# emrullahArkun/tinycarlo

Measured on AMD Instinct MI355X. Metric: env-steps/sec (whole node), higher is better.
Workload: dtype f64; 1 GPU; cfg3: 4096 envs/GPU, simple_layout map, 64x64 'classes' obs, with camera laneline raster; envs_per_gpu=4096, steps_per_launch=128, entry_point=tc_step_multi, observations=every step's frame stored to its own row of a [128, N, ...] rollout buffer, preroll_steps=1024, calls_prepared=True, actions=v~U(0.3,1) s~U(-1,1) maneuver~U{0..3}/64 steps, on device, autoreset=True, spawn=host queue (reference seed parity), resets_since_queue_top_up=18375, max_respawns_of_one_env_since_top_up=11, spawn_queue_len=64, max_segments_per_frame=49, frames_sampled=196608, on_road_term=False, lds_bytes_per_env=9760

## Files before the change

### tinycarlo_amd/csrc/k_common.h

```cpp
#ifndef K_COMMON_H
#define K_COMMON_H

#include <hip/hip_runtime.h>

#include "../../include/tinycarlo_hip.h"
#include "k_probe.h"
#include "tc_cull.h"
#include "tc_device.h"

#if defined(TC_PART) && defined(TC_DEV_FAST)
#error "the development builds are one translation unit"
#endif
#if defined(TC_PART) && TC_PART > 0
#define TC_PLAIN_KERNEL static
#else
#define TC_PLAIN_KERNEL
#endif

#define TC_PROF_RING 64
#define TC_RING_SLOTS 3
#define MODE_STEP 0
#define MODE_RESET 1
#define MODE_RENDER 2

__device__ __forceinline__ void lds_sync() { asm volatile("s_waitcnt lgkmcnt(0)" ::: "memory"); }

template <class T>
__device__ __forceinline__ const T& kernarg_again(const T& r) {
  unsigned long long p = (unsigned long long)&r;
  asm volatile("" : "+s"(p));
  return *(const T*)(const __attribute__((address_space(4))) T*)p;
}

#define RB_MAX 32
#define RB_OF_K(K) ((K) >= 8 ? 16 : 32)
#define R_OFF_TAB 0
#define R_TAB_BYTES_OF(RB) (((RB) * 4 * 5 + (RB) * 4 + 5 * (RB) + 8 * (RB)) * 4 + 2 * 4 * (RB) * 8)
#define R_OFF_BITS_OF(RB) ((R_TAB_BYTES_OF(RB) + 15) / 16 * 16)
#define R_OFF_LC_OF(RB) ((RB) * 116)
#define R_TAB_BYTES_SH(RB, sh) (R_OFF_LC_OF(RB) + ((RB) << (sh)) * (4 + 5 * 4))
#define R_OFF_BITS_SH(RB, sh) ((R_TAB_BYTES_SH(RB, sh) + 15) / 16 * 16)
static_assert(R_TAB_BYTES_SH(32, 2) == R_TAB_BYTES_OF(32) && R_TAB_BYTES_SH(16, 2) == R_TAB_BYTES_OF(16), "the four-edge form is the full size");
#define LCH 8

#define TC_MAX_GROUPS 8
struct LdsLayout {
  int off_p, off_flg, off_list, off_cnt;
  int total;
  int off_live;
};

struct LiveLds {
  double d[10];
  double cte, he, reward;
  double dist[TC_MAX_LAYERS];
  int lp[8];
  int lp_len, last_maneuver;
  int have_trig;
  int needs_reset;
  int cursor;
  int cursor0;
  int trunc, status, terminated;
  int ep_len;
  int cam_idx;
  int pad;
  int cnt[TC_MAX_TERMS];
  int ne[TC_MAX_LAYERS];
  double ep_ret;
};
#define TC_LIVE_BYTES 416
static_assert(sizeof(LiveLds) <= TC_LIVE_BYTES, "LiveLds must fit its LDS slot");

struct RollStep {
  double *reward, *cte, *heading_error;
  unsigned char *terminated, *truncated;
  int* status;
  double *x, *y, *theta, *velocity;
  double* dist;
  int* ne;
  int* lp;
  int* lp_len;
  size_t row0;
};

struct KArgs {
  DevMap m;
  DevCar car;
  DevCam cam;
  tc_buffers b;
  LdsLayout lds;
  int N;
  int env0;
  const double* cam_E;
  const double* cam_K;
  int* seg_g;
  int* seg_n;
  int seg_cap;
  const tc_term* terms;
  int n_terms;
  int* term_counters;
  int n_grp;
  int grp_layer[TC_MAX_GROUPS + 1];
  int grp_n0[TC_MAX_GROUPS + 1], grp_e0[TC_MAX_GROUPS + 1];
  int grp_l0[TC_MAX_GROUPS], grp_l1[TC_MAX_GROUPS];
  const double2* cam_nodes;
  const int2* cam_edges_g;
  int cap_nodes;
  const int* spawn_tab;
  int spawn_n;
  unsigned long long spawn_seed;
  unsigned int dbg;
  int seg_lds_off, seg_lds_cap;
  int clip_merge;
  int frame_cull;
  int cull_rows;
  const unsigned char* cull_tab;
  TcCullCover cull;
};

__device__ __forceinline__ double d_readlane(double v, int l) {
  const int lo = __builtin_amdgcn_readlane(__double2loint(v), l);
  const int hi = __builtin_amdgcn_readlane(__double2hiint(v), l);
  return __hiloint2double(hi, lo);
}

__device__ __forceinline__ int uni_i(int v) { return __builtin_amdgcn_readfirstlane(v); }
__device__ __forceinline__ double uni_d(double v) {
  const int lo = __builtin_amdgcn_readfirstlane(__double2loint(v));
  const int hi = __builtin_amdgcn_readfirstlane(__double2hiint(v));
  return __hiloint2double(hi, lo);
}

typedef __attribute__((address_space(3))) int* LdsIntPtr;

__device__ __forceinline__ int wave_rank(unsigned long long m) {
  return (int)__builtin_amdgcn_mbcnt_hi((unsigned)(m >> 32), __builtin_amdgcn_mbcnt_lo((unsigned)m, 0u));
}

__device__ inline unsigned int spread4(unsigned int x) {
  const unsigned int m = (x * 0x00204081u) & 0x01010101u;
  return (m << 8) - m;
}

__device__ __forceinline__ int wave_incl_scan(int v, int lane) {
  (void)lane;
  v += __builtin_amdgcn_update_dpp(0, v, 0x111, 0xf, 0xf, true);
  v += __builtin_amdgcn_update_dpp(0, v, 0x112, 0xf, 0xf, true);
  v += __builtin_amdgcn_update_dpp(0, v, 0x114, 0xf, 0xf, true);
  v += __builtin_amdgcn_update_dpp(0, v, 0x118, 0xf, 0xf, true);
  v += __builtin_amdgcn_update_dpp(0, v, 0x142, 0xa, 0xf, false);
  v += __builtin_amdgcn_update_dpp(0, v, 0x143, 0xc, 0xf, false);
  return v;
}

struct MultiArgs {
  int nsteps;
  int seg_rows;
  int cam_here;
  double* pose_rows;
  unsigned int* resident;
  int map_lds;
  int fat_lds;
  int grp_off, grp_stride, cnt_off;
  tc_rollout roll;
};
__device__ __forceinline__ RollStep roll_at(const tc_rollout& r, size_t row0, int C) {
  RollStep q;
  q.reward = r.reward;
  q.cte = r.cte;
  q.heading_error = r.heading_error;
  q.terminated = r.terminated;
  q.truncated = r.truncated;
  q.status = r.status;
  q.x = r.x;
  q.y = r.y;
  q.theta = r.theta;
  q.velocity = r.velocity;
  q.dist = r.laneline_distances;
  q.ne = r.nearest_edge;
  q.lp = r.local_path;
  q.lp_len = r.lp_len;
  q.row0 = row0;
  return q;
}

#endif
```

### tinycarlo_amd/csrc/k_raster.h

```cpp
#ifndef K_RASTER_H
#define K_RASTER_H

#include "k_common.h"
#include "tc_device.h"
#include "tc_rng.h"

struct RCam {
  int H, W, wpr, band_rows, n_bands, thickness, format;
  int cap_r;
  unsigned char cap_hw[32];
  unsigned int cap_hw4;
};
struct RArgs {
  int N, C;
  int env0;
  RCam cam;
  unsigned char colors[16][3];
  const int* seg_g;
  const int* seg_n;
  int seg_cap;
  unsigned char* obs;
  const unsigned char* mask;
  int off_tab, off_bits;
  unsigned int flags;
  int seg_row0;
  int noise_row0;
  long long obs_row_stride;
  int noise_blobs, noise_max_radius;
  const unsigned char* noise_hw;
  unsigned long long noise_seed;
  const unsigned int* noise_step;
  int seg_lds_off, seg_lds_cap;
  unsigned int colors_packed[16];
};

#ifndef TC_RASTER_WAVES
#define TC_RASTER_WAVES 4
#endif
#ifndef TC_BAND_VMCNT
#define TC_BAND_VMCNT 0
#endif
#define TC_BAND_THROTTLE() asm volatile("s_waitcnt vmcnt(%0)" ::"n"(TC_BAND_VMCNT) : "memory")
__host__ __device__ __forceinline__ size_t tc_obs_bytes_of(int fmt, int C, int H, int W) {
  return fmt == TC_FMT_CLASSES_BITS ? (size_t)C * H * (size_t)(W >> 3) : (size_t)H * W * (fmt == TC_FMT_CLASSES ? C : 3);
}
#define TC_FMT_IS_CLASSES(fmt) ((fmt) == TC_FMT_CLASSES || (fmt) == TC_FMT_CLASSES_BITS)
__device__ __forceinline__ void packed_zero_words(unsigned char* dst, const int nw, const int tid) {
  if ((((unsigned long long)dst) & 15ull) == 0) {
    const int n4 = nw >> 2;
    const uint4 z = make_uint4(0, 0, 0, 0);
    for (int q = tid; q < n4; q += TC_NT) ((uint4*)dst)[q] = z;
    for (int i = (n4 << 2) + tid; i < nw; i += TC_NT) ((unsigned int*)dst)[i] = 0u;
  } else {
    for (int i = tid; i < nw; i += TC_NT) ((unsigned int*)dst)[i] = 0u;
  }
}
__device__ __forceinline__ void packed_copy_words(unsigned char* dst, const unsigned int* src, const int src_word0, const int nw,
                                                  const int tid) {
  if ((((unsigned long long)dst) & 15ull) == 0 && (src_word0 & 3) == 0) {
    const int n4 = nw >> 2;
    for (int q = tid; q < n4; q += TC_NT) ((uint4*)dst)[q] = ((const uint4*)src)[q];
    for (int i = (n4 << 2) + tid; i < nw; i += TC_NT) ((unsigned int*)dst)[i] = src[i];
  } else {
    for (int i = tid; i < nw; i += TC_NT) ((unsigned int*)dst)[i] = src[i];
  }
}
template <bool THICK, int FMT, bool LDSONLY = false, int RB = RB_MAX, bool FORM = false, bool ONE_BAND = false>
__device__ __forceinline__ void raster_body(const RArgs& a0, unsigned char* smem, int env, unsigned char* obs_base,
                                            const int tid, const size_t seg_slot0, const int nseg_in,
                                            const unsigned int used_in, const int frame_row) {
  const RArgs& a = a0;
  const RCam& cam = a.cam;
  auto n_bands_of = [](const RCam& c) { return ONE_BAND ? 1 : c.n_bands; };
  unsigned int* bits = (unsigned int*)(smem + (FORM ? a.off_bits : R_OFF_BITS_OF(RB)));
  const int* segg = a.seg_g + (seg_slot0 + env) * a.seg_cap * 5;
  const LdsIntPtr seg_lds = (LdsIntPtr)(smem + a.seg_lds_off);
  const int seg_lds_cap = a.seg_lds_cap;
  struct SegV {
    int v[5];
    __device__ __forceinline__ int operator[](int i) const { return v[i]; }
  };
  int lds_base = 0;
  const bool refill = LDSONLY && nseg_in > seg_lds_cap;
  const int rb_step = (refill && seg_lds_cap < RB) ? seg_lds_cap : RB;
  auto seg_refill = [&](int base, int nb) {
    lds_sync();
    for (int i = threadIdx.x; i < 5 * nb; i += TC_NT) seg_lds[i] = segg[5 * base + i];
    lds_base = base;
    lds_sync();
  };
  auto seg_get = [&](int k) {
    SegV r;
    if (LDSONLY) {
#pragma unroll
      for (int i = 0; i < 5; i++) r.v[i] = seg_lds[5 * (k - lds_base) + i];
    } else if (k < seg_lds_cap) {
#pragma unroll
      for (int i = 0; i < 5; i++) r.v[i] = seg_lds[5 * k + i];
    } else {
#pragma unroll
      for (int i = 0; i < 5; i++) r.v[i] = segg[5 * k + i];
    }
    return r;
  };
  auto seg_layer = [&](int k) { return LDSONLY ? seg_lds[5 * (k - lds_base)] : k < seg_lds_cap ? seg_lds[5 * k] : segg[5 * k]; };
  int nseg = nseg_in;
  unsigned int used_layers = used_in;
  TSTAMP(8);
  if (!LDSONLY && nseg_in < 0) {
    nseg = a.seg_n[seg_slot0 + env];
    used_layers = 0;
    for (int k = tid; k < nseg; k += TC_NT) used_layers |= 1u << segg[5 * k];
#pragma unroll
    for (int off = 32; off > 0; off >>= 1) used_layers |= __shfl_xor(used_layers, off);
  }

  int H = cam.H, W = cam.W, wpr = cam.wpr, C = a.C;
  constexpr bool CLS = TC_FMT_IS_CLASSES(FMT), BITS = FMT == TC_FMT_CLASSES_BITS;
  unsigned char* out = obs_base + (size_t)env * tc_obs_bytes_of(FMT, C, H, W);
  int* lt0 = (int*)(smem + R_OFF_TAB);
  int* lc0 = lt0 + RB * 4 * 5;
  int* fl = FORM ? (int*)(smem + R_OFF_TAB) : lc0 + RB * 4;
  int* fc = fl + RB;
  int* fm = fc + RB;
  int* fd = fm + RB;
  int* fpy = fd + 2 * RB;
  int* fpv = fpy + 4 * RB;
  long long* fpx = (long long*)(fpv + 4 * RB);
  long long* fpd = fpx + 4 * RB;
  static_assert(R_OFF_LC_OF(RB) == 13 * RB * 4 + 2 * 4 * RB * 8 && (13 * RB * 4) % 8 == 0, "FORM: lc starts where the fixed tables end");
  unsigned int early_zero = 0;
  if (CLS && n_bands_of(cam) == 1 && (W & 15) == 0 && a.noise_blobs == 0 && !DBG_ON(a.flags, DBG_SKIP_STORE)) {
    const int per_plane = H * (W >> 4);
    const uint4 zero4 = make_uint4(0, 0, 0, 0);
    for (int c = 0; c < C; c++) {
      if ((used_layers >> c) & 1u) continue;
      if (BITS) {
        packed_zero_words(out + (size_t)c * H * wpr * 4, H * wpr, tid);
        continue;
      }
      uint4* po = (uint4*)(out + (size_t)c * H * W);
      for (int q = tid; q < per_plane; q += TC_NT) po[q] = zero4;
    }
    early_zero = ~used_layers;
    if (nseg == 0) {
      TSTAMP(9);
      TSTAMP(10);
      TSTAMP(11);
      TSTAMP(12);
      TSTAMP(13);
      TSTAMP_REAL(31);
      return;
    }
  }
  for (int band = 0; band < n_bands_of(cam); band++) {
    if constexpr (FORM && !ONE_BAND) {
      const RArgs& ab = kernarg_again(a0);
      H = ab.cam.H, W = ab.cam.W, wpr = ab.cam.wpr, C = ab.C;
    }
    const int y0 = band * cam.band_rows;
    const int y1 = (y0 + cam.band_rows < H) ? y0 + cam.band_rows : H;
    const int rows = y1 - y0;
    const int nwords = C * cam.band_rows * wpr;
    if (n_bands_of(cam) > 1 && (W & 15) == 0) {
      bool touched = refill;
      const long long mg = (long long)cam.thickness + 2;
      for (int k0 = 0; k0 < nseg && !touched; k0 += TC_NT) {
        bool t = false;
        if (k0 + tid < nseg) {
          const SegV sg = seg_get(k0 + tid);
          const long long ya = sg[2], yb = sg[4];
          t = (ya < yb ? yb : ya) + mg >= y0 && (ya < yb ? ya : yb) - mg < y1;
        }
        touched = __ballot(t) != 0;
      }
      if (!touched && DBG_ON(a.flags, DBG_SKIP_STORE)) continue;
      if (!touched) {
        const uint4 z = make_uint4(0, 0, 0, 0);
        TC_BAND_THROTTLE();
        if (BITS) {
          for (int c = 0; c < C; c++) packed_zero_words(out + ((size_t)c * H + y0) * wpr * 4, rows * wpr, tid);
        } else if (CLS) {
          const int per_plane = rows * (W >> 4);
          for (int c = 0; c < C; c++) {
            uint4* dst = (uint4*)(out + ((size_t)c * H + y0) * W);
            for (int q = tid; q < per_plane; q += TC_NT) dst[q] = z;
          }
        } else {
          const int n16 = rows * W * 3 / 16;
          uint4* dst = (uint4*)(out + (size_t)y0 * W * 3);
          for (int q = tid; q < n16; q += TC_NT) dst[q] = z;
        }
        continue;
      }
    }
    {
      const int n4 = nwords >> 2;
      for (int i = tid; i < n4; i += TC_NT) ((uint4*)bits)[i] = make_uint4(0, 0, 0, 0);
      for (int i = (n4 << 2) + tid; i < nwords; i += TC_NT) bits[i] = 0;
    }
    lds_sync();
    TSTAMP(9);
#ifdef TC_TIMING_LDS
    TSTAMP(26);
#endif
    Ras r;
    r.W = W;
    r.H = H;
    r.wpr = wpr;
    r.y0 = y0;
    r.y1 = y1;
    const int plane = cam.band_rows * wpr;
    if (DBG_ON(a.flags, DBG_SKIP_RASTER)) {
    } else if (!THICK) {
      for (int base = 0; base < nseg; base += refill ? rb_step : nseg) {
        const int nb = refill ? (nseg - base < rb_step ? nseg - base : rb_step) : nseg;
        if (refill) seg_refill(base, nb);
        for (int k = base + tid; k < base + nb; k += TC_NT) {
          const SegV sg = seg_get(k);
          r.bits = bits + sg[0] * plane;
          r_line_bresenham(r, sg[1], sg[2], sg[3], sg[4]);
        }
      }
    } else {
      for (int base = 0; base < nseg; base += rb_step) {
        const RArgs& a = kernarg_again(a0);
        const RCam& cam = a.cam;
        const int nb = nseg - base < rb_step ? nseg - base : rb_step;
        if (refill) seg_refill(base, nb);
#ifdef TC_TIMING_LDS
        if (cam.n_bands >= 0) TSTAMP(27);
#endif
        if (n_bands_of(cam) > 1) {
          bool t = false;
          if (tid < nb) {
            const SegV sg = seg_get(base + tid);
            const long long ya = sg[2], yb = sg[4], mg = (long long)cam.thickness + 2;
            t = (ya < yb ? yb : ya) + mg >= y0 && (ya < yb ? ya : yb) - mg < y1;
          }
          if (__ballot(t) == 0) continue;
        }
#ifdef TC_TIMING_LDS
        if (cam.thickness > 0) TSTAMP(24);
#endif
        if (tid < RB) {
          int nrow = 0, lo = 0, np = 0, wm = 0, dpx = 0, dpy = 0, okq = 0;
#ifdef TC_TIMING_LDS
          TSTAMP(25);
#endif
          if (tid < nb) {
            const SegV sg = seg_get(base + tid);
            long long qx0, qx1, qx2, qx3, qy0, qy1, qy2, qy3;
            TSTAMP(20);
            bool touch = true;
            if (n_bands_of(cam) > 1) {
              const long long ya = sg[2], yb = sg[4], mg = (long long)cam.thickness + 2;
              const long long ymin = (ya < yb ? ya : yb) - mg, ymax = (ya < yb ? yb : ya) + mg;
              touch = ymax >= y0 && ymin < y1;
            }
            if (touch && !DBG_ON(a.flags, DBG_SKIP_QUAD) && r_quad_dp(sg[1], sg[2], sg[3], sg[4], cam.thickness, dpx, dpy)) {
              TSTAMP(21);
              okq = 1;
              r_quad_vertices(sg[1], sg[2], sg[3], sg[4], dpx, dpy, qx0, qx1, qx2, qx3, qy0, qy1, qy2, qy3);
              int hi = -1;
              if (!DBG_ON(a.flags, DBG_SKIP_EVENTS))
              np = r_fill_events(W, H, qx0, qx1, qx2, qx3, qy0, qy1, qy2, qy3, fpy + 4 * tid, fpv + 4 * tid, wm, lo,
                                 hi);
              TSTAMP(22);
              if (lo < y0) lo = y0;
              if (hi > y1 - 1) hi = y1 - 1;
              if (np > 0 && hi >= lo) nrow = hi - lo + 1;
            }
          }
          fl[tid] = lo;
          fc[tid] = nrow;
          fm[tid] = np | (wm << 8) | (okq << 16);
          fd[2 * tid] = dpx;
          fd[2 * tid + 1] = dpy;
        }
        lds_sync();
        TSTAMP(10);
        MARK("outline setup");
        const int sh = (a.flags & R_F_LONG_EDGES) ? 1 : 2;
        const int n_items = FORM ? RB << sh : RB * 4;
        int* lc = FORM ? (int*)(fpd + 4 * RB) : lc0;
        int* lt = FORM ? lc + n_items : lt0;
        for (int t = tid; t < n_items; t += TC_NT) {
          int nchunk = 0;
          const int j = t >> sh;
          if (t < (nb << sh) && ((fm[j] >> 16) & 1)) {
            const int s0 = t & ((1 << sh) - 1), e = s0 << (2 - sh);
            const SegV sg = seg_get(base + j);
            const int dpx = fd[2 * j], dpy = fd[2 * j + 1];
            const int np = fm[j] & 0xff;
#pragma nounroll
            for (int h = 0; h < (8 >> sh) && !DBG_ON(a.flags, DBG_SKIP_SLOPE); h += 2) {
              const bool want = s0 + h < np;
              if (h != 0 && __ballot(want) == 0) break;
              if (want) {
                const int s = 4 * j + s0 + h;
                long long xs, dxs;
                r_fill_slope(sg[1], sg[2], sg[3], sg[4], dpx, dpy, fpy[s], fpv[s], xs, dxs);
                fpx[s] = xs;
                fpd[s] = dxs;
              }
            }
            LineP L;
            L.ecount = -1;
            if (!DBG_ON(a.flags, DBG_SKIP_LINESETUP)) L = r_outline_edge(W, H, sg[1], sg[2], sg[3], sg[4], dpx, dpy, e);
            if (L.ecount >= 0) {
              r.bits = bits + sg[0] * plane;
              r_put(r, L.ex, L.ey);
              int* o = lt + 5 * t;
              o[0] = L.a;
              o[1] = L.b;
              o[2] = L.step;
              o[3] = L.ecount | (L.xmajor << 30);
              o[4] = sg[0];
              nchunk = (L.ecount + LCH) / LCH;
            }
          }
          lc[t] = nchunk;
        }
        lds_sync();
        MARK("prefix sums");
        int tot_l, tot_f;
        {
          static_assert(RB * 4 == 2 * TC_NT || RB * 4 == TC_NT, "outline-edge chunk counts: one or two per lane");
          constexpr bool TWO = RB * 4 == 2 * TC_NT;
          const bool two = TWO && !(FORM && sh == 1);
          const bool mine = !FORM || tid < n_items;
          int v0 = two ? lc[2 * tid] : (mine ? lc[tid] : 0), v1 = two ? lc[2 * tid + 1] : 0;
          int inc = wave_incl_scan(v0 + v1, tid);
          tot_l = __builtin_amdgcn_readlane(inc, TC_NT - 1);
          int f = tid < RB ? fc[tid] : 0;
          int finc = wave_incl_scan(f, tid);
          tot_f = __builtin_amdgcn_readlane(finc, TC_NT - 1);
          if (two) {
            lc[2 * tid] = inc - v0 - v1;
            lc[2 * tid + 1] = inc - v1;
          } else if (mine) {
            lc[tid] = inc - v0;
          }
          if (tid < RB) fc[tid] = finc - f;
        }
        lds_sync();
        TSTAMP(11);
        for (int c = tid; c < tot_l && !DBG_ON(a.flags, DBG_SKIP_R2); c += TC_NT) {
          int lo = 0, hi = n_items;
          while (hi - lo > 1) {
            int mid = (lo + hi) >> 1;
            if (lc[mid] <= c) lo = mid; else hi = mid;
          }
          const int* o = lt + 5 * lo;
          const int ecount = o[3] & 0xffff, xmajor = (o[3] >> 30) & 1;
          const int k0 = (c - lc[lo]) * LCH;
          const int k1 = k0 + LCH - 1 < ecount ? k0 + LCH - 1 : ecount;
          r.bits = bits + o[4] * plane;
          r_line2_pixels(r, o[0], o[1], o[2], xmajor, k0, k1);
        }
        MARK("fill rows");
        for (int c = tid; c < tot_f && !DBG_ON(a.flags, DBG_SKIP_R3); c += TC_NT) {
          int lo = 0, hi = RB;
          while (hi - lo > 1) {
            int mid = (lo + hi) >> 1;
            if (fc[mid] <= c) lo = mid; else hi = mid;
          }
          const int row = fl[lo] + (c - fc[lo]);
          const int mm = fm[lo];
          r.bits = bits + seg_layer(base + lo) * plane;
          r_fill_row(r, row, mm & 0xff, (mm >> 8) & 0xff, fpy + 4 * lo, fpx + 4 * lo, fpd + 4 * lo);
        }
        MARK("caps");
        for (int t = tid; t < nb * 2 && !DBG_ON(a.flags, DBG_SKIP_R4); t += TC_NT) {
          const int k = base + (t >> 1);
          const SegV sg = seg_get(k);
          r.bits = bits + sg[0] * plane;
          const int cx = (t & 1) ? sg[3] : sg[1], cy = (t & 1) ? sg[4] : sg[2];
          if (n_bands_of(cam) > 1 && ((long long)cy + cam.cap_r < y0 || (long long)cy - cam.cap_r >= y1)) continue;
          if (cam.cap_r < 32)
            r_cap(r, cx, cy, cam.cap_r, cam.cap_hw, cam.cap_hw4);
          else
            r_circle_fill(r, cx, cy, cam.cap_r);
        }
        lds_sync();
      }
    }
    lds_sync();
    if (CLS && a.noise_blobs > 0) {
      const int nbl = a.noise_blobs, nb = C * nbl, mr = a.noise_max_radius;
      int* bp = (int*)(smem + R_OFF_TAB);
      unsigned char* bh = (unsigned char*)(bp + 2 * nb);
      const bool staged = nb * 8 + nb * rows <= (FORM ? a.off_bits : R_OFF_BITS_OF(RB)) - R_OFF_TAB;
      const unsigned int nstep = *a.noise_step + (unsigned int)frame_row;
      for (int k = tid; k < nb; k += TC_NT) {
        const tc_blob bl = tc_noise_blob(a.noise_seed, (uint32_t)env, nstep, (uint32_t)k, W, H, mr, C);
        bp[2 * k] = bl.x | (bl.y << 16);
        bp[2 * k + 1] = bl.r | (bl.mode << 12) | (bl.src << 16);
      }
      lds_sync();
      if (staged) {
        for (int row = tid; row < rows; row += TC_NT) {
#pragma unroll 5
          for (int k = 0; k < nb; k++) {
            const int by = bp[2 * k] >> 16, rr = bp[2 * k + 1] & 0xfff;
            int t = y0 + row - by;
            t = t < 0 ? -t : t;
            bh[k * rows + row] = t <= rr ? a.noise_hw[rr * mr + t] : (unsigned char)0;
          }
        }
        lds_sync();
      }
      const int items = rows * wpr;
      for (int it = tid; it < items; it += TC_NT) {
        const int row = it / wpr, w = it - row * wpr;
        const int yy = y0 + row, x_lo = w << 5;
        for (int c = 0; c < C; c++) {
          unsigned int cur = bits[(c * cam.band_rows + row) * wpr + w];
          for (int j = 0; j < nbl; j++) {
            const int k = c * nbl + j;
            const int p0 = bp[2 * k], p1 = bp[2 * k + 1];
            const int bx = p0 & 0xffff, by = p0 >> 16, rr = p1 & 0xfff, src = p1 >> 16;
            int t = yy - by;
            t = t < 0 ? -t : t;
            if (t <= rr) {
              const int hwv = staged ? (int)bh[k * rows + row] : (int)a.noise_hw[rr * mr + t];
              int xl = bx - hwv, xr = bx + hwv;
              xl = xl < 0 ? 0 : xl;
              xr = xr > W - 1 ? W - 1 : xr;
              const int b0 = xl > x_lo ? xl - x_lo : 0, b1 = xr < x_lo + 31 ? xr - x_lo : 31;
              if (b1 >= b0) {
                const unsigned int mask = (0xffffffffu >> (31 - b1)) & (0xffffffffu << b0);
                if ((p1 >> 12) & 1) {
                  const unsigned int sw = src == c ? cur : bits[(src * cam.band_rows + row) * wpr + w];
                  cur |= sw & mask;
                } else {
                  cur &= ~mask;
                }
              }
            }
          }
          bits[(c * cam.band_rows + row) * wpr + w] = cur;
        }
      }
      lds_sync();
      used_layers = C >= 32 ? 0xffffffffu : ((1u << C) - 1u);
    }
    TSTAMP(12);
    const RArgs& a = kernarg_again(a0);
    const RCam& cam = a.cam;
    if (n_bands_of(cam) > 1) TC_BAND_THROTTLE();
    if (DBG_ON(a.flags, DBG_SKIP_STORE)) {
    } else if (BITS) {
      for (int c = 0; c < C; c++) {
        if ((early_zero >> c) & 1u) continue;
        unsigned char* po = out + ((size_t)c * H + y0) * wpr * 4;
        const int w0 = c * cam.band_rows * wpr;
        if ((used_layers >> c) & 1u)
          packed_copy_words(po, bits + w0, w0, rows * wpr, tid);
        else
          packed_zero_words(po, rows * wpr, tid);
      }
    } else if (CLS) {
      if ((W & 15) == 0) {
        const int g = W >> 4;
        const int per_plane = rows * g;
        const bool dense = (W & 31) == 0;
        const uint4 zero4 = make_uint4(0, 0, 0, 0);
        for (int c = 0; c < C; c++) {
          const unsigned int* pl = bits + c * cam.band_rows * wpr;
          unsigned char* po = out + ((size_t)c * H + y0) * W;
          if ((early_zero >> c) & 1u) continue;
          if (!((used_layers >> c) & 1u)) {
            for (int q = tid; q < per_plane; q += TC_NT) *(uint4*)(po + (size_t)q * 16) = zero4;
            continue;
          }
          if (dense) {
            for (int q0 = tid; q0 < per_plane; q0 += 4 * TC_NT) {
              unsigned int w4[4];
#pragma unroll
              for (int j = 0; j < 4; j++) {
                const int q = q0 + j * TC_NT;
                w4[j] = q < per_plane ? pl[q >> 1] : 0u;
              }
#pragma unroll
              for (int j = 0; j < 4; j++) {
                const int q = q0 + j * TC_NT;
                const unsigned int b16 = (w4[j] >> ((q & 1) << 4)) & 0xffffu;
                uint4 o = zero4;
                if (__ballot(b16 != 0)) {
                  o.x = spread4(b16 & 15u);
                  o.y = spread4((b16 >> 4) & 15u);
                  o.z = spread4((b16 >> 8) & 15u);
                  o.w = spread4(b16 >> 12);
                }
                if (q < per_plane) *(uint4*)(po + (size_t)q * 16) = o;
              }
            }
            continue;
          }
          for (int q = tid; q < per_plane; q += TC_NT) {
            const int yy = q / g;
            const int xx = (q - yy * g) << 4;
            const unsigned int b16 = (pl[yy * wpr + (xx >> 5)] >> (xx & 31)) & 0xffffu;
            uint4 o = zero4;
            if (__ballot(b16 != 0)) {
              o.x = spread4(b16 & 15u);
              o.y = spread4((b16 >> 4) & 15u);
              o.z = spread4((b16 >> 8) & 15u);
              o.w = spread4(b16 >> 12);
            }
            *(uint4*)(po + (size_t)q * 16) = o;
          }
        }
      } else {
        const int per_plane = rows * W;
        const int total = C * per_plane;
        for (int q = tid; q < total; q += TC_NT) {
          int c = q / per_plane, p = q - c * per_plane;
          int yy = p / W, xx = p - yy * W;
          unsigned int word = bits[(c * cam.band_rows + yy) * wpr + (xx >> 5)];
          out[((size_t)c * H + y0 + yy) * W + xx] = ((word >> (xx & 31)) & 1u) ? 255 : 0;
        }
      }
    } else {
      if ((W & 15) == 0) {
        {
          const int n16 = rows * W * 3 / 16;
          uint4* dst = (uint4*)(out + (size_t)y0 * W * 3);
          const uint4 z = make_uint4(0, 0, 0, 0);
          for (int q = tid; q < n16; q += TC_NT) dst[q] = z;
        }
        const int nw = rows * wpr;
        const int pstride = cam.band_rows * wpr;
        const __attribute__((address_space(4))) unsigned int* pk =
            (const __attribute__((address_space(4))) unsigned int*)(unsigned long long)&a.colors_packed[0];
        for (int c = C - 1; c >= 0; c--) {
          const unsigned int col = pk[c];
          const unsigned char c0 = (unsigned char)col, c1 = (unsigned char)(col >> 8), c2 = (unsigned char)(col >> 16);
          for (int q = tid; q < nw; q += TC_NT) {
            unsigned int mine = bits[c * pstride + q];
            if (mine == 0) continue;
            for (int h = c + 1; h < C; h++) mine &= ~bits[h * pstride + q];
            const int yy = q / wpr, xw = (q - yy * wpr) << 5;
            unsigned char* row = out + ((size_t)(y0 + yy) * W + xw) * 3;
            while (mine) {
              const int bpos = __ffs(mine) - 1;
              mine &= mine - 1;
              unsigned char* o = row + bpos * 3;
              o[0] = c0;
              o[1] = c1;
              o[2] = c2;
            }
          }
        }
      } else if ((W & 3) == 0) {
        const int total = rows * W / 4;
        for (int g = tid; g < total; g += TC_NT) {
          int pix = g * 4;
          int yy = pix / W, xx = pix - yy * W;
          unsigned int top4 = 0;
          for (int c = 0; c < C; c++) {
            unsigned int word = bits[(c * cam.band_rows + yy) * wpr + (xx >> 5)];
            unsigned int m4 = spread4((word >> (xx & 31)) & 15u);
            top4 = (top4 & ~m4) | (m4 & (0x01010101u * (unsigned)(c + 1)));
          }
          unsigned char px[12];
#pragma unroll
          for (int k = 0; k < 4; k++) {
            int top = (int)((top4 >> (8 * k)) & 255u) - 1;
            px[3 * k] = top >= 0 ? a.colors[top][0] : 0;
            px[3 * k + 1] = top >= 0 ? a.colors[top][1] : 0;
            px[3 * k + 2] = top >= 0 ? a.colors[top][2] : 0;
          }
          unsigned int* o = (unsigned int*)(out + ((size_t)(y0 + yy) * W + xx) * 3);
          o[0] = px[0] | (px[1] << 8) | (px[2] << 16) | ((unsigned)px[3] << 24);
          o[1] = px[4] | (px[5] << 8) | (px[6] << 16) | ((unsigned)px[7] << 24);
          o[2] = px[8] | (px[9] << 8) | (px[10] << 16) | ((unsigned)px[11] << 24);
        }
      } else {
        const int total = rows * W;
        for (int p = tid; p < total; p += TC_NT) {
          int yy = p / W, xx = p - yy * W;
          int top = -1;
          for (int c = 0; c < C; c++) {
            unsigned int word = bits[(c * cam.band_rows + yy) * wpr + (xx >> 5)];
            if ((word >> (xx & 31)) & 1u) top = c;
          }
          unsigned char* o = out + ((size_t)(y0 + yy) * W + xx) * 3;
          o[0] = top >= 0 ? a.colors[top][0] : 0;
          o[1] = top >= 0 ? a.colors[top][1] : 0;
          o[2] = top >= 0 ? a.colors[top][2] : 0;
        }
      }
    }
    lds_sync();
  }
  TSTAMP(13);
  TSTAMP_REAL(31);
}

template <bool THICK, int FMT>
__global__ __launch_bounds__(TC_NT, TC_RASTER_WAVES) void tc_raster_kernel(RArgs a_unused) {
  extern __shared__ __align__(16) unsigned char smem[];
  const RArgs& a = *(const RArgs*)(const __attribute__((address_space(4))) RArgs*)__builtin_amdgcn_kernarg_segment_ptr();
  const int env = a.env0 + blockIdx.x;
  if (env >= a.N) return;
  if (a.mask && !a.mask[env]) return;
  const size_t slot0 = (size_t)(a.seg_row0 + blockIdx.y) * a.N;
  raster_body<THICK, FMT>(a, smem, env, a.obs + (size_t)blockIdx.y * a.obs_row_stride, threadIdx.x, slot0, -1, 0u, a.noise_row0 + (int)blockIdx.y);
}

#endif
```

Baseline: 185.2 million env-steps/s.

## Replace per-lane binary search with marker scatter and wave max-scan work dealing

In the FORM rasterizer path, outline-edge chunks and fill rows are now assigned to lanes by scattering a start marker (prefix<<7 | owner) into LDS and running a DPP inclusive max scan, instead of each lane binary-searching the prefix-sum array. The layer index is packed into existing words (o[3] and fm), which removes a separate load and the seg_layer lookup. This is meant to cut the LDS-bound, divergent binary-search loops. In exchange it adds an extra LDS round trip, a sync and a scan per 64-item pass. It also adds a host-side reference implementation of the dealing helpers.

```diff
diff --git a/tinycarlo_amd/csrc/k_common.h b/tinycarlo_amd/csrc/k_common.h
--- a/tinycarlo_amd/csrc/k_common.h
+++ b/tinycarlo_amd/csrc/k_common.h
@@ -153,6 +153,18 @@
   return v;
 }
 
+__device__ __forceinline__ int wave_incl_max(int x) {
+  unsigned int v = (unsigned int)x;
+  auto mx = [](unsigned int a, unsigned int b) { return a > b ? a : b; };
+  v = mx(v, (unsigned int)__builtin_amdgcn_update_dpp(0, (int)v, 0x111, 0xf, 0xf, true));
+  v = mx(v, (unsigned int)__builtin_amdgcn_update_dpp(0, (int)v, 0x112, 0xf, 0xf, true));
+  v = mx(v, (unsigned int)__builtin_amdgcn_update_dpp(0, (int)v, 0x114, 0xf, 0xf, true));
+  v = mx(v, (unsigned int)__builtin_amdgcn_update_dpp(0, (int)v, 0x118, 0xf, 0xf, true));
+  v = mx(v, (unsigned int)__builtin_amdgcn_update_dpp(0, (int)v, 0x142, 0xa, 0xf, false));
+  v = mx(v, (unsigned int)__builtin_amdgcn_update_dpp(0, (int)v, 0x143, 0xc, 0xf, false));
+  return (int)v;
+}
+
 struct MultiArgs {
   int nsteps;
   int seg_rows;
diff --git a/tinycarlo_amd/csrc/k_raster.h b/tinycarlo_amd/csrc/k_raster.h
--- a/tinycarlo_amd/csrc/k_raster.h
+++ b/tinycarlo_amd/csrc/k_raster.h
@@ -2,6 +2,7 @@
 #define K_RASTER_H
 
 #include "k_common.h"
+#include "tc_deal.h"
 #include "tc_device.h"
 #include "tc_rng.h"
 
@@ -244,12 +245,13 @@
         if (cam.thickness > 0) TSTAMP(24);
 #endif
         if (tid < RB) {
-          int nrow = 0, lo = 0, np = 0, wm = 0, dpx = 0, dpy = 0, okq = 0;
+          int nrow = 0, lo = 0, np = 0, wm = 0, dpx = 0, dpy = 0, okq = 0, layer = 0;
 #ifdef TC_TIMING_LDS
           TSTAMP(25);
 #endif
           if (tid < nb) {
             const SegV sg = seg_get(base + tid);
+            layer = sg[0];
             long long qx0, qx1, qx2, qx3, qy0, qy1, qy2, qy3;
             TSTAMP(20);
             bool touch = true;
@@ -274,7 +276,7 @@
           }
           fl[tid] = lo;
           fc[tid] = nrow;
-          fm[tid] = np | (wm << 8) | (okq << 16);
+          fm[tid] = np | (wm << 8) | (okq << 16) | (FORM ? layer << 17 : 0);
           fd[2 * tid] = dpx;
           fd[2 * tid + 1] = dpy;
         }
@@ -315,8 +317,12 @@
               o[0] = L.a;
               o[1] = L.b;
               o[2] = L.step;
-              o[3] = L.ecount | (L.xmajor << 30);
-              o[4] = sg[0];
+              if constexpr (FORM) {
+                o[3] = L.ecount | (sg[0] << 16) | (L.xmajor << 30);
+              } else {
+                o[3] = L.ecount | (L.xmajor << 30);
+                o[4] = sg[0];
+              }
               nchunk = (L.ecount + LCH) / LCH;
             }
           }
@@ -325,6 +331,7 @@
         lds_sync();
         MARK("prefix sums");
         int tot_l, tot_f;
+        int dl_p0 = 0, dl_n0 = 0, dl_p1 = 0, dl_n1 = 0, dl_t0 = 0, df_p = 0, df_n = 0;
         {
           static_assert(RB * 4 == 2 * TC_NT || RB * 4 == TC_NT, "outline-edge chunk counts: one or two per lane");
           constexpr bool TWO = RB * 4 == 2 * TC_NT;
@@ -336,40 +343,87 @@
           int f = tid < RB ? fc[tid] : 0;
           int finc = wave_incl_scan(f, tid);
           tot_f = __builtin_amdgcn_readlane(finc, TC_NT - 1);
-          if (two) {
-            lc[2 * tid] = inc - v0 - v1;
-            lc[2 * tid + 1] = inc - v1;
-          } else if (mine) {
-            lc[tid] = inc - v0;
-          }
-          if (tid < RB) fc[tid] = finc - f;
+          if constexpr (FORM) {
+            dl_t0 = two ? 2 * tid : tid;
+            dl_p0 = inc - v0 - v1, dl_n0 = v0, dl_p1 = inc - v1, dl_n1 = v1;
+            df_p = finc - f, df_n = f;
+          } else {
+            if (two) {
+              lc[2 * tid] = inc - v0 - v1;
+              lc[2 * tid + 1] = inc - v1;
+            } else if (mine) {
+              lc[tid] = inc - v0;
+            }
+            if (tid < RB) fc[tid] = finc - f;
+          }
         }
         lds_sync();
         TSTAMP(11);
-        for (int c = tid; c < tot_l && !DBG_ON(a.flags, DBG_SKIP_R2); c += TC_NT) {
-          int lo = 0, hi = n_items;
-          while (hi - lo > 1) {
-            int mid = (lo + hi) >> 1;
-            if (lc[mid] <= c) lo = mid; else hi = mid;
-          }
-          const int* o = lt + 5 * lo;
-          const int ecount = o[3] & 0xffff, xmajor = (o[3] >> 30) & 1;
-          const int k0 = (c - lc[lo]) * LCH;
-          const int k1 = k0 + LCH - 1 < ecount ? k0 + LCH - 1 : ecount;
-          r.bits = bits + o[4] * plane;
-          r_line2_pixels(r, o[0], o[1], o[2], xmajor, k0, k1);
-        }
-        MARK("fill rows");
-        for (int c = tid; c < tot_f && !DBG_ON(a.flags, DBG_SKIP_R3); c += TC_NT) {
-          int lo = 0, hi = RB;
-          while (hi - lo > 1) {
-            int mid = (lo + hi) >> 1;
-            if (fc[mid] <= c) lo = mid; else hi = mid;
-          }
-          const int row = fl[lo] + (c - fc[lo]);
-          const int mm = fm[lo];
-          r.bits = bits + seg_layer(base + lo) * plane;
-          r_fill_row(r, row, mm & 0xff, (mm >> 8) & 0xff, fpy + 4 * lo, fpx + 4 * lo, fpd + 4 * lo);
+        if constexpr (FORM) {
+          static_assert(!FORM || (RB == 32 && RB * 4 <= TC_DEAL_IDS && TC_NT == TC_DEAL_LANES), "lc holds >= 64 words and a marker names every entry");
+          auto deal = [&](const int c0, const int carry, const int p0, const int n0, const int t0, const int p1, const int n1) {
+            lc[tid] = 0;
+            if (tc_deal_starts(p0, n0, c0)) lc[p0 - c0] = tc_deal_word(p0, t0);
+            if (tc_deal_starts(p1, n1, c0)) lc[p1 - c0] = tc_deal_word(p1, t0 + 1);
+            lds_sync();
+            const int w = wave_incl_max(lc[tid]);
+            return w > carry ? w : carry;
+          };
+          int carry = 0;
+          for (int c0 = 0; c0 < tot_l && !DBG_ON(a.flags, DBG_SKIP_R2); c0 += TC_NT) {
+            const int w = deal(c0, carry, dl_p0, dl_n0, dl_t0, dl_p1, dl_n1);
+            carry = __builtin_amdgcn_readlane(w, TC_NT - 1);
+            const int c = c0 + tid;
+            if (c < tot_l) {
+              const int* o = lt + 5 * tc_deal_owner(w);
+              const int o3 = o[3];
+              const int ecount = o3 & 0xffff, xmajor = (o3 >> 30) & 1;
+              const int k0 = tc_deal_offset(w, c) * LCH;
+              const int k1 = k0 + LCH - 1 < ecount ? k0 + LCH - 1 : ecount;
+              r.bits = bits + ((o3 >> 16) & 31) * plane;
+              r_line2_pixels(r, o[0], o[1], o[2], xmajor, k0, k1);
+            }
+          }
+          MARK("fill rows");
+          carry = 0;
+          for (int c0 = 0; c0 < tot_f && !DBG_ON(a.flags, DBG_SKIP_R3); c0 += TC_NT) {
+            const int w = deal(c0, carry, df_p, df_n, tid, 0, 0);
+            carry = __builtin_amdgcn_readlane(w, TC_NT - 1);
+            const int c = c0 + tid;
+            if (c < tot_f) {
+              const int lo = tc_deal_owner(w);
+              const int row = fl[lo] + tc_deal_offset(w, c);
+              const int mm = fm[lo];
+              r.bits = bits + ((mm >> 17) & 31) * plane;
+              r_fill_row(r, row, mm & 0xff, (mm >> 8) & 0xff, fpy + 4 * lo, fpx + 4 * lo, fpd + 4 * lo);
+            }
+          }
+        } else {
+          for (int c = tid; c < tot_l && !DBG_ON(a.flags, DBG_SKIP_R2); c += TC_NT) {
+            int lo = 0, hi = n_items;
+            while (hi - lo > 1) {
+              int mid = (lo + hi) >> 1;
+              if (lc[mid] <= c) lo = mid; else hi = mid;
+            }
+            const int* o = lt + 5 * lo;
+            const int ecount = o[3] & 0xffff, xmajor = (o[3] >> 30) & 1;
+            const int k0 = (c - lc[lo]) * LCH;
+            const int k1 = k0 + LCH - 1 < ecount ? k0 + LCH - 1 : ecount;
+            r.bits = bits + o[4] * plane;
+            r_line2_pixels(r, o[0], o[1], o[2], xmajor, k0, k1);
+          }
+          MARK("fill rows");
+          for (int c = tid; c < tot_f && !DBG_ON(a.flags, DBG_SKIP_R3); c += TC_NT) {
+            int lo = 0, hi = RB;
+            while (hi - lo > 1) {
+              int mid = (lo + hi) >> 1;
+              if (fc[mid] <= c) lo = mid; else hi = mid;
+            }
+            const int row = fl[lo] + (c - fc[lo]);
+            const int mm = fm[lo];
+            r.bits = bits + seg_layer(base + lo) * plane;
+            r_fill_row(r, row, mm & 0xff, (mm >> 8) & 0xff, fpy + 4 * lo, fpx + 4 * lo, fpd + 4 * lo);
+          }
         }
         MARK("caps");
         for (int t = tid; t < nb * 2 && !DBG_ON(a.flags, DBG_SKIP_R4); t += TC_NT) {
diff --git a/tinycarlo_amd/csrc/tc_deal.h b/tinycarlo_amd/csrc/tc_deal.h
--- /dev/null
+++ b/tinycarlo_amd/csrc/tc_deal.h
@@ -0,0 +1,45 @@
+#ifndef TC_DEAL_H
+#define TC_DEAL_H
+#include "tc_trig.h"
+
+#define TC_DEAL_BITS 7
+#define TC_DEAL_IDS (1 << TC_DEAL_BITS)
+#define TC_DEAL_LANES 64
+
+TC_HD int tc_deal_word(int pre, int t) { return (pre << TC_DEAL_BITS) | t; }
+TC_HD int tc_deal_owner(int w) { return w & (TC_DEAL_IDS - 1); }
+TC_HD int tc_deal_offset(int w, int c) { return c - (int)((unsigned)w >> TC_DEAL_BITS); }
+TC_HD int tc_deal_starts(int pre, int cnt, int c0) { return cnt != 0 && (unsigned)(pre - c0) < (unsigned)TC_DEAL_LANES; }
+
+TC_HD int tc_deal_search(const int* pre, int n, int c) {
+  int lo = 0, hi = n;
+  while (hi - lo > 1) {
+    const int mid = (lo + hi) >> 1;
+    if (pre[mid] <= c) lo = mid; else hi = mid;
+  }
+  return lo;
+}
+
+TC_HD void tc_deal_scan64(int* w) {
+  int s[TC_DEAL_LANES];
+  for (int d = 1; d < 16; d <<= 1) {
+    for (int l = 0; l < TC_DEAL_LANES; l++) s[l] = (l & 15) >= d ? w[l - d] : 0;
+    for (int l = 0; l < TC_DEAL_LANES; l++) w[l] = w[l] > s[l] ? w[l] : s[l];
+  }
+  for (int l = 0; l < TC_DEAL_LANES; l++) s[l] = ((l >> 4) & 1) ? w[(l & ~15) - 1] : 0;
+  for (int l = 0; l < TC_DEAL_LANES; l++) w[l] = w[l] > s[l] ? w[l] : s[l];
+  for (int l = 0; l < TC_DEAL_LANES; l++) s[l] = l >= 32 ? w[31] : 0;
+  for (int l = 0; l < TC_DEAL_LANES; l++) w[l] = w[l] > s[l] ? w[l] : s[l];
+}
+
+TC_HD int tc_deal_pass(const int* pre, const int* cnt, int n, int c0, int carry, int* scratch, int* words) {
+  for (int l = 0; l < TC_DEAL_LANES; l++) scratch[l] = 0;
+  for (int t = 0; t < n; t++)
+    if (tc_deal_starts(pre[t], cnt[t], c0)) scratch[pre[t] - c0] = tc_deal_word(pre[t], t);
+  for (int l = 0; l < TC_DEAL_LANES; l++) words[l] = scratch[l];
+  tc_deal_scan64(words);
+  for (int l = 0; l < TC_DEAL_LANES; l++) words[l] = words[l] > carry ? words[l] : carry;
+  return words[TC_DEAL_LANES - 1];
+}
+
+#endif
```

After: 189.1 million env-steps/s (median of 6 runs). 1.02x the previous value.
